# calledit/metric_depth_video_toolbox

Measured on AMD Instinct MI355X. Metric: stereo frames/sec at 1920x1080 (+ achieved HBM GB/s vs roofline), higher is better.
Workload: dtype u8/f32; 1 GPU; 1920x1080 stereo reproject, 65 mm baseline, xfov 45, points mode, 128 distinct frames per step per GPU, inputs resident in HBM (BASELINE.json configs[1] shape, batched past the 256 MiB Infinity Cache); distinct_gpus=1, ranks_seen_by_the_process_group=1

## Files before the change

metric_depth_video_toolbox_amd/csrc/mdvt_edge_filter.hip:

```cpp
#include "mdvt_device.h"

namespace mdvt {


__device__ __forceinline__ bool tri_oblique(const double (&a)[3], const double (&b)[3], const double (&c)[3])
{
    const double e1x = b[0] - a[0], e1y = b[1] - a[1], e1z = b[2] - a[2];
    const double e2x = c[0] - a[0], e2y = c[1] - a[1], e2z = c[2] - a[2];
    const double nx = e1y * e2z - e1z * e2y;
    const double ny = e1z * e2x - e1x * e2z;
    const double nz = e1x * e2y - e1y * e2x;
    const double vx = -((a[0] + b[0]) + c[0]) / 3.0;
    const double vy = -((a[1] + b[1]) + c[1]) / 3.0;
    const double vz = -((a[2] + b[2]) + c[2]) / 3.0;
    const double dot = (nx * vx + ny * vy) + nz * vz;
    const double len_n = sqrt((nx * nx + ny * ny) + nz * nz);
    const double len_v = sqrt((vx * vx + vy * vy) + vz * vz);
    const double cosine = dot / (len_n * len_v + 1e-15);
    return cosine < 0x1.1df0b2b89dd37p-6;
}

constexpr double kScreenMargin = 1e-6;
constexpr double kScreenMinNNSS = 9e-16;

__device__ __forceinline__ int tri_oblique_screen(const double (&a)[3], const double (&b)[3], const double (&c)[3])
{
    const double e1x = b[0] - a[0], e1y = b[1] - a[1], e1z = b[2] - a[2];
    const double e2x = c[0] - a[0], e2y = c[1] - a[1], e2z = c[2] - a[2];
    const double nx = fma(e1y, e2z, -(e1z * e2y));
    const double ny = fma(e1z, e2x, -(e1x * e2z));
    const double nz = fma(e1x, e2y, -(e1y * e2x));
    const double sx = (a[0] + b[0]) + c[0], sy = (a[1] + b[1]) + c[1], sz = (a[2] + b[2]) + c[2];
    const double d = -fma(nz, sz, fma(ny, sy, nx * sx));
    const double nn = fma(nz, nz, fma(ny, ny, nx * nx));
    const double ss = fma(sz, sz, fma(sy, sy, sx * sx));
    const double c0 = 0x1.1df0b2b89dd37p-6;
    const double rhs = (c0 * c0) * (nn * ss);
    if (!(nn * ss > kScreenMinNNSS)) return 2;
    const double lhs = d * fabs(d);
    const double tol = kScreenMargin * rhs;
    if (lhs < rhs - tol) return 1;
    if (lhs > rhs + tol) return 0;
    return 2;
}

__device__ __forceinline__ int tri_oblique_screen_f32(float a, float b, float pp, float z0, float t12 ,
                                                      float nx, float ny, float sx, float sy, float sz)
{
    const float nz = -__builtin_fmaf(a, nx, __builtin_fmaf(b, ny, t12));
    const float nn = __builtin_fmaf(nz, nz, __builtin_fmaf(ny, ny, nx * nx));
    const float ss = __builtin_fmaf(sz, sz, __builtin_fmaf(sy, sy, sx * sx));
    const float d3 = (3.0f * z0) * t12;
    const float lhs = d3 * d3;
    const float nnss = nn * ss;
    const float rhs = 0x1.3f61d0p-12f * nnss;
    const bool ok = nnss > 1.0e-15f;
    const bool rem = ok && lhs < rhs * 0.999f, val = ok && lhs > rhs * 1.001f;
    return rem ? 1 : (val ? 0 : 2);
}

struct CellRaysF32 { float a, a1, b, b1, px, py; bool ok; };
__device__ __forceinline__ CellRaysF32 cell_rays_f32(double x0r, double x1r, double y0r, double y1r)
{
    CellRaysF32 r;
    r.a = (float)x0r; r.b = (float)y0r; r.a1 = (float)x1r; r.b1 = (float)y1r;
    r.px = (float)(x1r - x0r); r.py = (float)(y1r - y0r);
    r.ok = fabsf(r.a) <= 64.0f && fabsf(r.b) <= 64.0f && fabsf(r.a1) <= 64.0f && fabsf(r.b1) <= 64.0f;
    return r;
}

__device__ __forceinline__ uint32_t edge_filter_prescreen(const CellRaysF32& r, float zA, float zB, float zC, float zD)
{
    if (!r.ok) return 2u | (2u << 2);
    const float pp = r.px * r.py;
    const int s1 = tri_oblique_screen_f32(r.a, r.b, pp, zA, (pp * zB) * zC, (r.py * zA) * (zC - zB), (r.px * zC) * (zB - zA),
                                          __builtin_fmaf(r.a1, zC, r.a * (zA + zB)), __builtin_fmaf(r.b1, zB + zC, r.b * zA), (zA + zB) + zC);
    const int s2 = tri_oblique_screen_f32(r.a, r.b, pp, zA, (pp * zC) * zD, (r.py * zC) * (zD - zA), (r.px * zA) * (zC - zD),
                                          __builtin_fmaf(r.a1, zC + zD, r.a * zA), __builtin_fmaf(r.b1, zC, r.b * (zA + zD)), (zA + zC) + zD);
    return (uint32_t)s1 | ((uint32_t)s2 << 2);
}

__device__ __forceinline__ uint32_t edge_filter_cell(const FrameDev& f, int i, int j, int of_by_one, double x0r, double x1r, double y0r,
                                                     double y1r, uint32_t pre, float zA, float zB, float zC, float zD)
{
    int s1 = (int)(pre & 3u), s2 = (int)(pre >> 2);
    if (s1 == 2 || s2 == 2) {
        asm volatile("; f64 screen" ::: "memory");
        const double dA = (double)zA, dB = (double)zB, dC = (double)zC, dD = (double)zD;
        const double A[3] = {x0r * dA, y0r * dA, dA};
        const double B[3] = {x0r * dB, y1r * dB, dB};
        const double Cc[3] = {x1r * dC, y1r * dC, dC};
        const double D[3] = {x1r * dD, y0r * dD, dD};
        if (s1 == 2) s1 = tri_oblique_screen(A, B, Cc);
        if (s2 == 2) s2 = tri_oblique_screen(A, Cc, D);
    }
    if (s1 == 2 || s2 == 2) {
        double Ae[3], Be[3], Ce[3], De[3];
        vertex_f64(f, i, j, of_by_one, zA, Ae);
        vertex_f64(f, i + 1, j, of_by_one, zB, Be);
        vertex_f64(f, i + 1, j + 1, of_by_one, zC, Ce);
        vertex_f64(f, i, j + 1, of_by_one, zD, De);
        if (s1 == 2) s1 = tri_oblique(Ae, Be, Ce) ? 1 : 0;
        if (s2 == 2) s2 = tri_oblique(Ae, Ce, De) ? 1 : 0;
    }
    return (s1 == 1 ? 1u : 0u) | (s2 == 1 ? 2u : 0u);
}

__device__ __forceinline__ void edge_filter_mark_unused(uint8_t* u, int W, int i, int j, uint32_t inv)
{
    const size_t a = (size_t)i * W + j;
    u[a] = 1;
    u[a + W + 1] = 1;
    if (inv & 1u) u[a + W] = 1;
    if (inv & 2u) u[a + 1] = 1;
}

__global__ void __launch_bounds__(128) k_edge_filter(const uint8_t* __restrict__ depth_rgb, size_t pitch, size_t stride,
                              const FrameDev* __restrict__ fp, int frame0, int W, int H, int of_by_one,
                              float sx, float sy,
                              uint8_t* __restrict__ tri_invalid, size_t tri_stride,
                              uint8_t* __restrict__ unused, size_t unused_stride)
{
    const int j = blockIdx.x * blockDim.x + threadIdx.x;
    const int i = blockIdx.y;
    const int fr = blockIdx.z;
    if (j >= W - 1 || i >= H - 1) return;
    const uint8_t* r0 = depth_rgb + (size_t)(frame0 + fr) * stride + (size_t)i * pitch;
    const uint8_t* r1 = r0 + pitch;
    const uint32_t pA = load_px_bytes(r0, j), pD = load_px_bytes(r0, j + 1);
    const uint32_t pB = load_px_bytes(r1, j), pC = load_px_bytes(r1, j + 1);
    FrameDev f = fp[frame0 + fr];
    f.sx = sx; f.sy = sy;
    const float zA = decode_z(code16_of(pA), f.mult, f.scale);
    const float zD = decode_z(code16_of(pD), f.mult, f.scale);
    const float zB = decode_z(code16_of(pB), f.mult, f.scale);
    const float zC = decode_z(code16_of(pC), f.mult, f.scale);
    const double rfx = f.rKd[0], rfy = f.rKd[1];
    const double x0 = (of_by_one ? (double)((float)j * f.sx) : (double)j) - f.Kd[2];
    const double x1 = (of_by_one ? (double)((float)(j + 1) * f.sx) : (double)(j + 1)) - f.Kd[2];
    const double y0 = (of_by_one ? (double)((float)i * f.sy) : (double)i) - f.Kd[3];
    const double y1 = (of_by_one ? (double)((float)(i + 1) * f.sy) : (double)(i + 1)) - f.Kd[3];
    const double x0r = x0 * rfx, x1r = x1 * rfx, y0r = y0 * rfy, y1r = y1 * rfy;
    const uint32_t inv = edge_filter_cell(f, i, j, of_by_one, x0r, x1r, y0r, y1r, edge_filter_prescreen(cell_rays_f32(x0r, x1r, y0r, y1r), zA, zB, zC, zD), zA, zB, zC, zD);
    const size_t ncell = (size_t)(W - 1) * (H - 1);
    const size_t cell = (size_t)i * (W - 1) + j;
    if (tri_invalid) {
        uint8_t* t = tri_invalid + (size_t)fr * tri_stride;
        t[cell] = inv & 1u;
        t[ncell + cell] = (inv >> 1) & 1u;
    }
    if (unused && inv) edge_filter_mark_unused(unused + (size_t)fr * unused_stride, W, i, j, inv);
}

typedef uint32_t u32_unaligned_t __attribute__((aligned(1)));
__global__ void __launch_bounds__(128) k_edge_filter4(const uint8_t* __restrict__ depth_rgb, size_t pitch, size_t stride,
                              const FrameDev* __restrict__ fp, int frame0, int W, int H, int of_by_one,
                              float sx, float sy,
                              uint8_t* __restrict__ tri_invalid, size_t tri_stride,
                              uint8_t* __restrict__ unused, size_t unused_stride)
{
    const int g = blockIdx.x * blockDim.x + threadIdx.x;
    const int i = blockIdx.y;
    const int fr = blockIdx.z;
    const int j0 = 4 * g;
    if (j0 >= W - 1 || i >= H - 1) return;
    const uint32_t* r0 = (const uint32_t*)(depth_rgb + (size_t)(frame0 + fr) * stride + (size_t)i * pitch) + 3 * g;
    const uint32_t* r1 = (const uint32_t*)((const uint8_t*)r0 + pitch);
    const bool five = j0 + 4 < W;
    uint32_t p0[5], p1[5];
    unpack4(r0[0], r0[1], r0[2], *(uint32_t(*)[4])p0);
    unpack4(r1[0], r1[1], r1[2], *(uint32_t(*)[4])p1);
    p0[4] = five ? r0[3] & 0xFFFFFFu : 0u;
    p1[4] = five ? r1[3] & 0xFFFFFFu : 0u;
    FrameDev f = fp[frame0 + fr];
    f.sx = sx; f.sy = sy;
    float z0[5], z1[5];
#pragma unroll
    for (int q = 0; q < 5; ++q) {
        z0[q] = decode_z(code16_of(p0[q]), f.mult, f.scale);
        z1[q] = decode_z(code16_of(p1[q]), f.mult, f.scale);
    }
    const double rfx = f.rKd[0], rfy = f.rKd[1];
    const double y0r = ((of_by_one ? (double)((float)i * f.sy) : (double)i) - f.Kd[3]) * rfy;
    const double y1r = ((of_by_one ? (double)((float)(i + 1) * f.sy) : (double)(i + 1)) - f.Kd[3]) * rfy;
    double xr[5];
#pragma unroll
    for (int q = 0; q < 5; ++q) xr[q] = ((of_by_one ? (double)((float)(j0 + q) * f.sx) : (double)(j0 + q)) - f.Kd[2]) * rfx;
    const int ncells = five ? 4 : 3;
    float fx[5];
    const float fb = (float)y0r, fb1 = (float)y1r, fpy = (float)(y1r - y0r);
    bool rays_ok = fabsf(fb) <= 64.0f && fabsf(fb1) <= 64.0f;
#pragma unroll
    for (int q = 0; q < 5; ++q) { fx[q] = (float)xr[q]; rays_ok = rays_ok && fabsf(fx[q]) <= 64.0f; }
    uint32_t w1 = 0, w2 = 0, any = 0;
    uint32_t inv[4] = {0, 0, 0, 0}, pre[4] = {0, 0, 0, 0};
    uint32_t und = 0;
#pragma unroll
    for (int q = 0; q < 4; ++q) {
        if (q < ncells) {
            CellRaysF32 r;
            r.a = fx[q]; r.a1 = fx[q + 1]; r.b = fb; r.b1 = fb1; r.px = (float)(xr[q + 1] - xr[q]); r.py = fpy;
            r.ok = rays_ok;
            pre[q] = edge_filter_prescreen(r, z0[q], z1[q], z1[q + 1], z0[q + 1]);
        }
        und |= pre[q] & 0xAu;
        inv[q] = (pre[q] & 1u) | ((pre[q] >> 1) & 2u);
    }
    if (und) {
#pragma unroll
        for (int q = 0; q < 4; ++q)
            if (pre[q] & 0xAu) inv[q] = edge_filter_cell(f, i, j0 + q, of_by_one, xr[q], xr[q + 1], y0r, y1r, pre[q], z0[q], z1[q], z1[q + 1], z0[q + 1]);
    }
#pragma unroll
    for (int q = 0; q < 4; ++q) {
        w1 |= (inv[q] & 1u) << (8 * q);
        w2 |= ((inv[q] >> 1) & 1u) << (8 * q);
        any |= inv[q];
    }
    const size_t ncell = (size_t)(W - 1) * (H - 1);
    const size_t cell = (size_t)i * (W - 1) + j0;
    if (tri_invalid) {
        uint8_t* t = tri_invalid + (size_t)fr * tri_stride;
        if (five) {
            *(u32_unaligned_t*)(t + cell) = w1;
            *(u32_unaligned_t*)(t + ncell + cell) = w2;
        } else {
#pragma unroll
            for (int q = 0; q < 3; ++q) { t[cell + q] = (w1 >> (8 * q)) & 1u; t[ncell + cell + q] = (w2 >> (8 * q)) & 1u; }
        }
    }
    if (unused && any) {
        uint8_t* u = unused + (size_t)fr * unused_stride;
#pragma unroll
        for (int q = 0; q < 4; ++q) if (inv[q]) edge_filter_mark_unused(u, W, i, j0 + q, inv[q]);
    }
}

hipError_t launch_edge_filter(const uint8_t* depth_rgb, size_t pitch, size_t stride, const FrameDev* fp, int frame0,
                              int n, int W, int H, int of_by_one, uint8_t* tri_invalid, size_t tri_stride,
                              uint8_t* unused, size_t unused_stride, hipStream_t s)
{
    const float sx = of_by_one ? (float)(((double)W + 1.0) / (double)W) : 1.0f;
    const float sy = of_by_one ? (float)(((double)H + 1.0) / (double)H) : 1.0f;
    const bool dwords = W % 4 == 0 && W >= 8 && pitch % 4 == 0 && stride % 4 == 0 && ((uintptr_t)depth_rgb % 4) == 0;
    if (dwords) {
        dim3 grid((W / 4 + 127) / 128, H - 1, n);
        hipLaunchKernelGGL(k_edge_filter4, grid, dim3(128), 0, s, depth_rgb, pitch, stride, fp, frame0, W, H, of_by_one,
                           sx, sy, tri_invalid, tri_stride, unused, unused_stride);
    } else {
        dim3 grid((W - 1 + 127) / 128, H - 1, n);
        hipLaunchKernelGGL(k_edge_filter, grid, dim3(128), 0, s, depth_rgb, pitch, stride, fp, frame0, W, H, of_by_one,
                           sx, sy, tri_invalid, tri_stride, unused, unused_stride);
    }
    return hipGetLastError();
}

}
```

Baseline: 218,100 stereo frames/s.

## Band edge-filter rows, add a float smoothness fast path, compact slow cells across the wave

Each thread now walks a band of four cell rows and keeps the lower row's decoded depths in registers, so each depth row is loaded and decoded roughly once instead of twice. A cheap float bound built from the intrinsics decides whether a cell's four depths are smooth enough to pass without the full test. Cells that fail it are compacted through LDS with ballot/mbcnt so all lanes of the wave share the expensive double-precision edge_filter_cell work, which reduces divergence. The cost is LDS traffic and wave barriers, fewer blocks per launch, and reliance on the smoothness bound being conservative so results stay exact.

```diff
diff --git a/metric_depth_video_toolbox_amd/csrc/mdvt_edge_filter.hip b/metric_depth_video_toolbox_amd/csrc/mdvt_edge_filter.hip
--- a/metric_depth_video_toolbox_amd/csrc/mdvt_edge_filter.hip
+++ b/metric_depth_video_toolbox_amd/csrc/mdvt_edge_filter.hip
@@ -152,87 +152,165 @@
     if (unused && inv) edge_filter_mark_unused(unused + (size_t)fr * unused_stride, W, i, j, inv);
 }
 
+struct SmoothBound { float tau, zfloor; bool ok; };
+__device__ __forceinline__ SmoothBound edge_filter_smooth_bound(const FrameDev& f, int W, int H, int of_by_one)
+{
+    const float fxf = (float)f.Kd[0], fyf = (float)f.Kd[1], cx = (float)f.Kd[2], cy = (float)f.Kd[3];
+    const float px = (float)f.rKd[0], py = (float)f.rKd[1];
+    const float xl = of_by_one ? (float)(W - 1) * f.sx : (float)(W - 1);
+    const float yl = of_by_one ? (float)(H - 1) * f.sy : (float)(H - 1);
+    const float U = fmaxf(fabsf(cx), fabsf(xl - cx)) * px, V = fmaxf(fabsf(cy), fabsf(yl - cy)) * py;
+    const float G1 = ((1.0f + U) * fxf + (1.0f + V) * fyf) + 1.0f;
+    const float rrho = __builtin_amdgcn_rsqf((1.0f + U * U) + V * V);
+    SmoothBound b;
+    b.tau = fminf(0.015625f, (44.0f * rrho - 1.0f) * __builtin_amdgcn_rcpf(G1));
+    b.zfloor = 1.01f * __builtin_amdgcn_exp2f(__builtin_amdgcn_logf((1e-13f * fxf) * fyf) * (1.0f / 3.0f));
+    b.ok = px > 0.0f && py > 0.0f && U <= 64.0f && V <= 64.0f && b.tau > 0.0f && b.zfloor > 0.0f;
+    if (!b.ok) { b.tau = -1.0f; b.zfloor = __builtin_inff(); }
+    return b;
+}
+
+__device__ __forceinline__ bool edge_filter_cell_smooth(const SmoothBound& b, float zA, float zB, float zC, float zD)
+{
+    const int iA = __float_as_int(zA), iB = __float_as_int(zB), iC = __float_as_int(zC), iD = __float_as_int(zD);
+    const float lo = __int_as_float(min(min(iA, iB), min(iC, iD))), hi = __int_as_float(max(max(iA, iB), max(iC, iD)));
+    return (int)(lo >= b.zfloor) & (int)(hi - lo <= b.tau * lo);
+}
+
+__device__ __forceinline__ void wave_lds_sync()
+{
+    __builtin_amdgcn_fence(__ATOMIC_RELEASE, "wavefront");
+    __builtin_amdgcn_wave_barrier();
+    __builtin_amdgcn_fence(__ATOMIC_ACQUIRE, "wavefront");
+}
+
 typedef uint32_t u32_unaligned_t __attribute__((aligned(1)));
+constexpr int kEdgeBandRows = 4;
+
+__device__ __forceinline__ void edge_filter_load_row(const uint8_t* row, int g, bool live, bool five, uint32_t (&w)[4])
+{
+    w[0] = w[1] = w[2] = w[3] = 0u;
+    if (live) {
+        const uint32_t* r = (const uint32_t*)row + 3 * g;
+        w[0] = r[0]; w[1] = r[1]; w[2] = r[2];
+        if (five) w[3] = r[3];
+    }
+}
+
+__device__ __forceinline__ void edge_filter_decode_row(const uint32_t (&w)[4], float mult, float scale, float (&z)[5])
+{
+    uint32_t p[5];
+    unpack4(w[0], w[1], w[2], *(uint32_t(*)[4])p);
+    p[4] = w[3] & 0xFFFFFFu;
+#pragma unroll
+    for (int q = 0; q < 5; ++q) z[q] = decode_z(code16_of(p[q]), mult, scale);
+}
+
 __global__ void __launch_bounds__(128) k_edge_filter4(const uint8_t* __restrict__ depth_rgb, size_t pitch, size_t stride,
                               const FrameDev* __restrict__ fp, int frame0, int W, int H, int of_by_one,
                               float sx, float sy,
                               uint8_t* __restrict__ tri_invalid, size_t tri_stride,
                               uint8_t* __restrict__ unused, size_t unused_stride)
 {
+    __shared__ float s_z[2][10][64];
+    __shared__ uint32_t s_item[2][256];
     const int g = blockIdx.x * blockDim.x + threadIdx.x;
-    const int i = blockIdx.y;
+    const int i0 = blockIdx.y * kEdgeBandRows;
     const int fr = blockIdx.z;
     const int j0 = 4 * g;
-    if (j0 >= W - 1 || i >= H - 1) return;
-    const uint32_t* r0 = (const uint32_t*)(depth_rgb + (size_t)(frame0 + fr) * stride + (size_t)i * pitch) + 3 * g;
-    const uint32_t* r1 = (const uint32_t*)((const uint8_t*)r0 + pitch);
-    const bool five = j0 + 4 < W;
-    uint32_t p0[5], p1[5];
-    unpack4(r0[0], r0[1], r0[2], *(uint32_t(*)[4])p0);
-    unpack4(r1[0], r1[1], r1[2], *(uint32_t(*)[4])p1);
-    p0[4] = five ? r0[3] & 0xFFFFFFu : 0u;
-    p1[4] = five ? r1[3] & 0xFFFFFFu : 0u;
+    if (i0 >= H - 1) return;
+    const int nrows = min(kEdgeBandRows, H - 1 - i0);
+    const bool live = j0 < W - 1;
+    const bool five = live && j0 + 4 < W;
+    const uint32_t cells = live ? (five ? 15u : 7u) : 0u;
+    const uint8_t* rows = depth_rgb + (size_t)(frame0 + fr) * stride + (size_t)i0 * pitch;
+    uint32_t wu[4], wl[4], wn[4] = {0, 0, 0, 0};
+    edge_filter_load_row(rows, g, live, five, wu);
+    edge_filter_load_row(rows + pitch, g, live, five, wl);
     FrameDev f = fp[frame0 + fr];
     f.sx = sx; f.sy = sy;
+    const SmoothBound sb = edge_filter_smooth_bound(f, W, H, of_by_one);
+    const uint32_t lane = threadIdx.x & 63u;
+    float (*sz)[64] = s_z[threadIdx.x >> 6];
+    uint32_t* item = s_item[threadIdx.x >> 6];
+    const size_t ncell = (size_t)(W - 1) * (H - 1);
+    uint8_t* const t = tri_invalid ? tri_invalid + (size_t)fr * tri_stride : nullptr;
     float z0[5], z1[5];
-#pragma unroll
-    for (int q = 0; q < 5; ++q) {
-        z0[q] = decode_z(code16_of(p0[q]), f.mult, f.scale);
-        z1[q] = decode_z(code16_of(p1[q]), f.mult, f.scale);
-    }
-    const double rfx = f.rKd[0], rfy = f.rKd[1];
-    const double y0r = ((of_by_one ? (double)((float)i * f.sy) : (double)i) - f.Kd[3]) * rfy;
-    const double y1r = ((of_by_one ? (double)((float)(i + 1) * f.sy) : (double)(i + 1)) - f.Kd[3]) * rfy;
-    double xr[5];
-#pragma unroll
-    for (int q = 0; q < 5; ++q) xr[q] = ((of_by_one ? (double)((float)(j0 + q) * f.sx) : (double)(j0 + q)) - f.Kd[2]) * rfx;
-    const int ncells = five ? 4 : 3;
-    float fx[5];
-    const float fb = (float)y0r, fb1 = (float)y1r, fpy = (float)(y1r - y0r);
-    bool rays_ok = fabsf(fb) <= 64.0f && fabsf(fb1) <= 64.0f;
-#pragma unroll
-    for (int q = 0; q < 5; ++q) { fx[q] = (float)xr[q]; rays_ok = rays_ok && fabsf(fx[q]) <= 64.0f; }
-    uint32_t w1 = 0, w2 = 0, any = 0;
-    uint32_t inv[4] = {0, 0, 0, 0}, pre[4] = {0, 0, 0, 0};
-    uint32_t und = 0;
-#pragma unroll
-    for (int q = 0; q < 4; ++q) {
-        if (q < ncells) {
-            CellRaysF32 r;
-            r.a = fx[q]; r.a1 = fx[q + 1]; r.b = fb; r.b1 = fb1; r.px = (float)(xr[q + 1] - xr[q]); r.py = fpy;
-            r.ok = rays_ok;
-            pre[q] = edge_filter_prescreen(r, z0[q], z1[q], z1[q + 1], z0[q + 1]);
+    edge_filter_decode_row(wu, f.mult, f.scale, z0);
+    for (int r = 0; r < nrows; ++r) {
+        const int i = i0 + r;
+        if (r + 1 < nrows) edge_filter_load_row(rows + (size_t)(r + 2) * pitch, g, live, five, wn);
+        edge_filter_decode_row(wl, f.mult, f.scale, z1);
+        uint32_t und = 0;
+#pragma unroll
+        for (int q = 0; q < 4; ++q) und |= edge_filter_cell_smooth(sb, z0[q], z1[q], z1[q + 1], z0[q + 1]) ? 0u : 1u << q;
+        und &= cells;
+        uint32_t inv[4] = {0, 0, 0, 0};
+        if (__builtin_amdgcn_ballot_w64(und != 0) != 0) {
+            asm volatile("; gather" ::: "memory");
+#pragma unroll
+            for (int q = 0; q < 5; ++q) { sz[q][lane] = z0[q]; sz[5 + q][lane] = z1[q]; }
+            uint32_t pos[4], total = 0;
+#pragma unroll
+            for (int q = 0; q < 4; ++q) {
+                const bool mine = (und >> q) & 1u;
+                const uint64_t m = __builtin_amdgcn_ballot_w64(mine);
+                pos[q] = total + __builtin_amdgcn_mbcnt_hi((uint32_t)(m >> 32), __builtin_amdgcn_mbcnt_lo((uint32_t)m, 0u));
+                total += (uint32_t)__builtin_popcountll(m);
+                if (mine) item[pos[q]] = lane * 4u + (uint32_t)q;
+            }
+            wave_lds_sync();
+            const double rfx = f.rKd[0], rfy = f.rKd[1];
+            const double y0r = ((of_by_one ? (double)((float)i * f.sy) : (double)i) - f.Kd[3]) * rfy;
+            const double y1r = ((of_by_one ? (double)((float)(i + 1) * f.sy) : (double)(i + 1)) - f.Kd[3]) * rfy;
+            for (uint32_t base = 0; base < total; base += 64u) {
+                const uint32_t k = base + lane;
+                if (k < total) {
+                    const uint32_t it = item[k], owner = it >> 2, q = it & 3u;
+                    const float zA = sz[q][owner], zD = sz[q + 1u][owner], zB = sz[5u + q][owner], zC = sz[6u + q][owner];
+                    const int j = 4 * (g - (int)lane + (int)owner) + (int)q;
+                    const double x0r = ((of_by_one ? (double)((float)j * f.sx) : (double)j) - f.Kd[2]) * rfx;
+                    const double x1r = ((of_by_one ? (double)((float)(j + 1) * f.sx) : (double)(j + 1)) - f.Kd[2]) * rfx;
+                    item[k] = edge_filter_cell(f, i, j, of_by_one, x0r, x1r, y0r, y1r,
+                                               edge_filter_prescreen(cell_rays_f32(x0r, x1r, y0r, y1r), zA, zB, zC, zD), zA, zB, zC, zD);
+                }
+            }
+            wave_lds_sync();
+#pragma unroll
+            for (int q = 0; q < 4; ++q)
+                if ((und >> q) & 1u) inv[q] = item[pos[q]];
+#pragma unroll
+            for (int q = 0; q < 5; ++q) z1[q] = sz[5 + q][lane];
+            wave_lds_sync();
         }
-        und |= pre[q] & 0xAu;
-        inv[q] = (pre[q] & 1u) | ((pre[q] >> 1) & 2u);
-    }
-    if (und) {
-#pragma unroll
-        for (int q = 0; q < 4; ++q)
-            if (pre[q] & 0xAu) inv[q] = edge_filter_cell(f, i, j0 + q, of_by_one, xr[q], xr[q + 1], y0r, y1r, pre[q], z0[q], z1[q], z1[q + 1], z0[q + 1]);
-    }
-#pragma unroll
-    for (int q = 0; q < 4; ++q) {
-        w1 |= (inv[q] & 1u) << (8 * q);
-        w2 |= ((inv[q] >> 1) & 1u) << (8 * q);
-        any |= inv[q];
-    }
-    const size_t ncell = (size_t)(W - 1) * (H - 1);
-    const size_t cell = (size_t)i * (W - 1) + j0;
-    if (tri_invalid) {
-        uint8_t* t = tri_invalid + (size_t)fr * tri_stride;
-        if (five) {
-            *(u32_unaligned_t*)(t + cell) = w1;
-            *(u32_unaligned_t*)(t + ncell + cell) = w2;
-        } else {
-#pragma unroll
-            for (int q = 0; q < 3; ++q) { t[cell + q] = (w1 >> (8 * q)) & 1u; t[ncell + cell + q] = (w2 >> (8 * q)) & 1u; }
+        if (live) {
+            uint32_t w1 = 0, w2 = 0, any = 0;
+#pragma unroll
+            for (int q = 0; q < 4; ++q) {
+                w1 |= (inv[q] & 1u) << (8 * q);
+                w2 |= ((inv[q] >> 1) & 1u) << (8 * q);
+                any |= inv[q];
+            }
+            const size_t cell = (size_t)i * (W - 1) + j0;
+            if (t) {
+                if (five) {
+                    *(u32_unaligned_t*)(t + cell) = w1;
+                    *(u32_unaligned_t*)(t + ncell + cell) = w2;
+                } else {
+#pragma unroll
+                    for (int q = 0; q < 3; ++q) { t[cell + q] = (w1 >> (8 * q)) & 1u; t[ncell + cell + q] = (w2 >> (8 * q)) & 1u; }
+                }
+            }
+            if (unused && any) {
+                uint8_t* u = unused + (size_t)fr * unused_stride;
+#pragma unroll
+                for (int q = 0; q < 4; ++q) if (inv[q]) edge_filter_mark_unused(u, W, i, j0 + q, inv[q]);
+            }
         }
-    }
-    if (unused && any) {
-        uint8_t* u = unused + (size_t)fr * unused_stride;
-#pragma unroll
-        for (int q = 0; q < 4; ++q) if (inv[q]) edge_filter_mark_unused(u, W, i, j0 + q, inv[q]);
+#pragma unroll
+        for (int q = 0; q < 5; ++q) z0[q] = z1[q];
+#pragma unroll
+        for (int q = 0; q < 4; ++q) wl[q] = wn[q];
     }
 }
 
@@ -244,7 +322,7 @@
     const float sy = of_by_one ? (float)(((double)H + 1.0) / (double)H) : 1.0f;
     const bool dwords = W % 4 == 0 && W >= 8 && pitch % 4 == 0 && stride % 4 == 0 && ((uintptr_t)depth_rgb % 4) == 0;
     if (dwords) {
-        dim3 grid((W / 4 + 127) / 128, H - 1, n);
+        dim3 grid((W / 4 + 127) / 128, (H - 1 + kEdgeBandRows - 1) / kEdgeBandRows, n);
         hipLaunchKernelGGL(k_edge_filter4, grid, dim3(128), 0, s, depth_rgb, pitch, stride, fp, frame0, W, H, of_by_one,
                            sx, sy, tri_invalid, tri_stride, unused, unused_stride);
     } else {
```

Result: slower. 209,800 stereo frames/s (-3.8%).
